# UCF-CRCV/TeD-SPAD

Measured on AMD Instinct MI355X. Metric: clips/sec (16x224^2 I3D features), higher is better.
Workload: dtype f16; 1 GPU; cfg2 dali_extraction path: largei3d extract_features, 225 clip times x 10 crops = 2250 clip-forwards of 3x16x224x224 per GPU per step, random-init weights; global_batch=375, parallelism=clip-sharded x1 + RCCL all-gather of (T,10,F) features

## Files before the change

### ted_spad_amd/csrc/conv_stem_pt.hip

```cpp
#include "conv_common.h"

namespace tedspad {
namespace {

__device__ uint4 g_zero16s;

typedef unsigned u32x4 __attribute__((ext_vector_type(4)));

constexpr int PT_TH = 8, PT_TW = 16;
constexpr int PT_PP = PT_TW + 3;
constexpr int PT_ROWB = 2 * PT_PP * 32;
constexpr int PT_NTAP = 49;
constexpr int PT_W_BYTES = PT_NTAP * 64 * 32;
constexpr int PT_REC = 48;
__host__ __device__ constexpr int pt_rows(int par) { return par == 0 ? PT_TH + 3 : PT_TH + 2; }
__host__ __device__ constexpr int pt_frame(int par) { return pt_rows(par) * PT_ROWB; }
__host__ __device__ constexpr int pt_jobs(int par) { return (2 * pt_frame(par) + 1023) / 1024; }
__host__ __device__ constexpr int pt_off(int par) { return par == 0 ? 0 : pt_jobs(0) * 1024; }
constexpr int PT_W_OFF = pt_off(1) + pt_jobs(1) * 1024;
constexpr int PT_LDS = PT_W_OFF + PT_W_BYTES;
constexpr int PT_NPAIR = 25;
constexpr int PT_W16_BYTES = PT_NPAIR * 64 * 64;
__host__ __device__ constexpr int pt_wbytes(int mf) { return mf == 16 ? PT_W16_BYTES : PT_W_BYTES; }
constexpr int PT_XB_ROW = 9 * 128, PT_XB_BYTES = PT_TH * PT_XB_ROW;
__host__ __device__ constexpr int pt_xb_off(int mf) { return PT_W_OFF + pt_wbytes(mf); }
__host__ __device__ constexpr int pt_lds_pool(int mf) { return pt_xb_off(mf) + PT_XB_BYTES; }
constexpr int PT_LDS_POOL = pt_lds_pool(32);
static_assert(pt_lds_pool(16) <= 160 * 1024 && pt_xb_off(16) % 128 == 0 && pt_xb_off(32) % 128 == 0, "MF = 16 image: exactly 160 KB");
constexpr int PT_POOL_PIECES = 4 * 9 * 8;
static_assert(PT_LDS_POOL <= 160 * 1024, "weights + halo (+ pooled rows) must fit the CU's LDS");
static_assert(PT_W_BYTES % 1024 == 0 && (4 * PT_ROWB) % 256 == 0 && PT_ROWB % 32 == 0, "LDS image alignment");

struct StemPT {
    const unsigned char *x;
    const unsigned char *wimg;
    const float *scale, *shift;
    uint16_t *y;
    long sTp;
    int sH, sP;
    int N, Tp, H, Wq, Ho, Wo, ldy, relu;
// ... 55 lines not shown
        for (int r = 0; r < 2; ++r)
#pragma unroll
            for (int f = 0; f < 2; ++f) xa[r * 2 + f] = *reinterpret_cast<const uint4 *>(dsm + pb[bi] + (pt_off(PAR) + off + f * FR + r * 4 * PT_ROWB));
#pragma unroll
        for (int cb = 0; cb < 2; ++cb) xw[cb] = *reinterpret_cast<const uint4 *>(dsm + wa + (PBASE + i) * 4096 + cb * 1024);
    };
    load(0, fx[0], fw[0]);
    __builtin_amdgcn_sched_group_barrier(0x100, 6, 0);
#pragma unroll
    for (int i = 0; i < NP; ++i) {
        if (i + 1 < NP) load(i + 1, fx[(i + 1) & 1], fw[(i + 1) & 1]);
#pragma unroll
        for (int cb = 0; cb < 2; ++cb)
#pragma unroll
            for (int r = 0; r < 2; ++r)
#pragma unroll
                for (int f = 0; f < 2; ++f) acc[cb][r][f] = T::mfma16(fw[i & 1][cb], fx[i & 1][r * 2 + f], acc[cb][r][f]);
        if (i + 1 < NP) __builtin_amdgcn_sched_group_barrier(0x100, 3, 0);
        __builtin_amdgcn_sched_group_barrier(0x008, 4, 0);
        if (i + 1 < NP) __builtin_amdgcn_sched_group_barrier(0x100, 3, 0);
        __builtin_amdgcn_sched_group_barrier(0x008, 4, 0);
    }
}

template <typename T, int NW, bool POOL, int MF = 32, bool DIRECT = false, int LW = 0>
__global__ __launch_bounds__(64 * (NW + LW)) void conv_stem_pt_kernel(const StemPT p) {
    static_assert(MF == 32 || (MF == 16 && NW == 8 && POOL), "the 16x16x32 form is built for 8 waves with the pool fused");
    static_assert(!DIRECT || (MF == 16 && NW == 8 && POOL), "the fp32-clip loader is built for the production form");
    static_assert(LW == 0 || (MF == 16 && NW == 8 && POOL), "loader waves are built for the production forms");
    constexpr int NA = NW == 8 ? 1 : 2;
    constexpr int XB_OFF = pt_xb_off(MF);
    constexpr int NPT = 64 * (LW ? LW : NW);
    constexpr int PIT = (PT_POOL_PIECES + NPT - 1) / NPT;
    constexpr int NTK = LW ? (4 * pt_rows(0) * 10 + NPT - 1) / NPT : 1;
    constexpr int NLW = LW ? LW : NW;
    constexpr int ROUNDS = (pt_jobs(0) + NLW - 1) / NLW;
    extern __shared__ __attribute__((aligned(16))) unsigned char dsm[];
    const int tid = threadIdx.x, lane = tid & 63;
    const int wave = __builtin_amdgcn_readfirstlane(tid >> 6);
    const int ptid = LW ? tid - 64 * NW : tid;
    const unsigned lds0 = (unsigned)(uintptr_t)(lptr_t)dsm;
    const unsigned char *zero = reinterpret_cast<const unsigned char *>(&g_zero16s);

    const int xcd = blockIdx.x & 7, nx = gridDim.x >> 3;
    const int base = xcd * p.chunk;
    const int lim = min(p.chunk, p.total - base);
    int k = blockIdx.x >> 3;
    if (k >= lim) return;

    if (wave < NW)
        for (int j = wave; j < pt_wbytes(MF) / 1024; j += NW) lds_dma16(p.wimg + j * 1024 + lane * 16, lds0 + PT_W_OFF + j * 1024);

    int off[2][ROUNDS], rc[2][ROUNDS];
    const int dw0 = LW ? wave - NW : wave;
    auto setup_dma = [&]() {
#pragma unroll
    for (int par = 0; par < 2; ++par)
#pragma unroll
        for (int i = 0; i < ROUNDS; ++i) {
            const int s = (i * NLW + dw0) * 64 + lane;
            const int hs = s & 1;
            int q = s >> 1;
            const int pos = q % PT_PP; q /= PT_PP;
            const int b = q & 1; q >>= 1;
            const int row = q % pt_rows(par), f = q / pt_rows(par);
            const int hr = 2 * row + par;
            const int hf = MF == 16 ? hs : hs ^ ((pos >> 3) & 1);
            const bool ok = f < 2;
            off[par][i] = ok ? f * 12 + hf * 16 + hr * p.sH + b * p.sP + (pos - 2) * PT_REC : 0;
            rc[par][i] = ok ? (hr << 8) | pos : (1 << 28);
        }
    };
    if (!DIRECT && !LW) setup_dma();
// ... 8 lines not shown
    auto locate = [&](Patch &q) {
        q.ho0 = q.th * PT_TH; q.wo0 = q.tw * PT_TW;
        q.ih0 = 2 * q.ho0 - 3; q.wqm2 = q.wo0 - 2;
        if (DIRECT) q.pf = p.xf + (long)q.n * p.sN + (long)(4 * q.tp - p.pad_t) * p.sT + (long)q.ih0 * p.sHf + (2 * q.wo0 - 4);
        else q.pb = p.x + ((long)q.n * p.Tp + q.tp) * p.sTp + (long)q.ih0 * p.sH + (long)q.wo0 * PT_REC;
    };
    int dn, dtp, dth, dtw;
    split(nx, dn, dtp, dth, dtw);
    auto advance = [&](const Patch &c) {
        Patch q = c;
        if (POOL && c.th + 1 < p.tiles_h) {
            ++q.th;
            locate(q);
            return q;
        }
        if (POOL) q.th = 0;
        q.tw += dtw; if (q.tw >= p.tiles_w) { q.tw -= p.tiles_w; if (POOL) ++q.tp; else ++q.th; }
        if (!POOL) { q.th += dth; if (q.th >= p.tiles_h) { q.th -= p.tiles_h; ++q.tp; } }
        q.tp += dtp; if (q.tp >= p.Tp) { q.tp -= p.Tp; ++q.n; }
        q.n += dn;
        locate(q);
        return q;
    };
    auto issue = [&](int par, const Patch &q) {
#pragma unroll
        for (int i = 0; i < ROUNDS; ++i) {
            const int j = i * NLW + dw0;
            if (j >= pt_jobs(par)) break;
            const bool ok = (unsigned)(q.ih0 + (rc[par][i] >> 8)) < (unsigned)p.H && (unsigned)(q.wqm2 + (rc[par][i] & 255)) < (unsigned)p.Wq;
            lds_dma16(ok ? q.pb + off[par][i] : zero, lds0 + pt_off(par) + j * 1024);
        }
    };

    int so[2][NTK][LW ? 1 : 8], fsch[2][NTK][2], ldst[2][NTK], dcol[2][NTK], drow[2][NTK];
    f32x4 stage[2][NTK][8];
    auto setup_tasks = [&]() {
#pragma unroll
        for (int par = 0; par < 2; ++par)
#pragma unroll
            for (int t = 0; t < NTK; ++t) {
                const int tk = ptid + t * NPT;
                const int per = pt_rows(par) * 10;
                const int fh = tk / per, rem = tk - fh * per;
                const int row = rem / 10, q4c = rem - row * 10;
                const int f = fh >> 1, hs = fh & 1, hr = 2 * row + par;
                const bool task = fh < 4;
                drow[par][t] = task ? hr : (1 << 20);
                dcol[par][t] = 4 * q4c;
                ldst[par][t] = task ? pt_off(par) + f * pt_frame(par) + row * PT_ROWB + 2 * q4c * 32 + 16 * hs : -1;
                if (LW) { drow[par][t] = (task ? hr : 4095) | (4 * q4c) << 12 | (fh & 3) << 20; dcol[par][t] = 0; so[par][t][0] = hr * p.sHf + 4 * q4c; }
                fsch[par][t][0] = fsch[par][t][1] = 0;
#pragma unroll
                for (int e = 0; e < 8; ++e) {
                    const int v = 6 * f + 8 * hs + e, fs = v / 3, ch = v - 3 * fs;
                    if (!LW) so[par][t][e] = ch * p.sC + fs * p.sT + hr * p.sHf + 4 * q4c;
                    fsch[par][t][e >> 2] |= (fs | (ch << 3)) << (8 * (e & 3));
                }
            }
    };
    if (DIRECT && !LW) setup_tasks();
    auto ldst_of = [&](int par, int t) -> int {
        return ldst[par][t];
    };
    auto issue_d = [&](int par, const Patch &q) {
        const int tt0 = 4 * q.tp - p.pad_t;
#pragma unroll
        for (int t = 0; t < NTK; ++t) {
            int fc0 = fsch[par][t][0], fc1 = fsch[par][t][1], meta = drow[par][t], sb = so[par][t][0];
            if (LW) asm volatile("" : "+v"(meta), "+v"(sb), "+v"(fc0), "+v"(fc1));
            const int t_row = LW ? meta & 4095 : drow[par][t], t_col = LW ? (meta >> 12) & 255 : dcol[par][t];
            const bool rowok = (unsigned)(q.ih0 + t_row) < (unsigned)p.H && (unsigned)(2 * q.wo0 - 4 + t_col) < (unsigned)p.W;
            const bool hs1 = LW ? (t_row != 4095 && ((meta >> 20) & 1)) : (ldst[par][t] >= 0 && ((ldst[par][t] >> 4) & 1));
#pragma unroll
            for (int e = 0; e < 8; ++e) {
                const int code = ((e < 4 ? fc0 : fc1) >> (8 * (e & 3))) & 255;
                const bool ok = rowok && (unsigned)(tt0 + (code & 7)) < (unsigned)p.T && (code >> 3) < p.C && !(e == 7 && hs1);
                const int o = LW ? sb + (code >> 3) * p.sC + (code & 7) * p.sT : so[par][t][e];
                const float *src = ok ? q.pf + o : reinterpret_cast<const float *>(zero);
                unsigned long sa = reinterpret_cast<unsigned long>(src);
                asm volatile("" : "+v"(sa));
                stage[par][t][e] = *reinterpret_cast<const __attribute__((address_space(1))) f32x4 *>(sa);
            }
        }
        asm volatile("" ::: "memory");
    };
    auto cvt2 = [&](float a, float b) -> unsigned {
        if constexpr (T::kDtype == TEDSPAD_F16) {
            unsigned pk;
            const float x = __builtin_amdgcn_fmed3f(a, -65504.f, 65504.f), y = __builtin_amdgcn_fmed3f(b, -65504.f, 65504.f);
            asm("v_cvt_pk_f16_f32 %0, %1, %2" : "=v"(pk) : "v"(x), "v"(y));
            return pk;
        } else {
            return (unsigned)T::from_f32(a) | ((unsigned)T::from_f32(b) << 16);
        }
    };
    auto pack_d = [&](int buf, int t, int j) -> uint4 {
        return make_uint4(cvt2(stage[buf][t][0][j], stage[buf][t][1][j]), cvt2(stage[buf][t][2][j], stage[buf][t][3][j]),
                          cvt2(stage[buf][t][4][j], stage[buf][t][5][j]), cvt2(stage[buf][t][6][j], stage[buf][t][7][j]));
    };
    auto write_d = [&](int par, int t, int j, uint4 v) {
        const bool last = (LW ? (drow[par][t] >> 12) & 255 : dcol[par][t]) == 36;
        const int la = ldst_of(par, t);
        if (la >= 0 && (j < 2 || !last)) *reinterpret_cast<uint4 *>(dsm + la + (j >> 1) * 32 + (j & 1) * (PT_PP * 32)) = v;
    };
    auto commit_d = [&](int par) {
#pragma unroll
        for (int t = 0; t < NTK; ++t)
#pragma unroll
            for (int j = 0; j < 4; ++j) write_d(par, t, j, pack_d(par, t, j));
    };
    Patch cur;
    split(base + k, cur.n, cur.tp, cur.th, cur.tw);
    locate(cur);
    if (DIRECT && !LW) {
        issue_d(0, cur);
        issue_d(1, cur);
        commit_d(0);
        commit_d(1);
    } else if (!DIRECT && !LW) {
        issue(0, cur);
        issue(1, cur);
    }

    auto successor = [&](const Patch &c, int kc, Patch &out, int &kout) -> bool {
        const bool wrap = !POOL || c.th + 1 == p.tiles_h;
        kout = wrap ? kc + nx : kc;
        out = c;
        if (kout >= lim) return false;
        out = advance(c);
        return true;
    };
    const bool dma = !(p.dbg & 1);
    int pxo[PIT], pi[PIT], psl[PIT];
    uint4 carry[PIT];
#pragma unroll
    for (int it = 0; it < PIT; ++it) {
        const int u = ptid + it * NPT;
        psl[it] = (u >> 3) % 9;
        pi[it] = (u >= 0 && u < PT_POOL_PIECES) ? (u >> 3) / 9 : -1;
        pxo[it] = XB_OFF + psl[it] * 128 + (u & 7) * 16;
        carry[it] = make_uint4(0, 0, 0, 0);
    }
    auto pool_rows = [&](const Patch &q) {
        const size_t fr = (size_t)q.n * p.Tp + q.tp;
#pragma unroll
        for (int it = 0; it < PIT; ++it) {
            if (LW) {
                int u = ptid + it * NPT;
                asm volatile("" : "+v"(u));
                psl[it] = (u >> 3) % 9;
                pi[it] = u < PT_POOL_PIECES ? (u >> 3) / 9 : -1;
                pxo[it] = XB_OFF + psl[it] * 128 + (u & 7) * 16;
// ... 20 lines not shown


    if (LW && !DIRECT && wave >= NW) {
        setup_dma();
        Patch c = cur, n1 = cur;
        int kc = k, k1 = 0;
        issue(0, c);
        issue(1, c);
        wait_vmcnt<0>();
        __builtin_amdgcn_s_barrier();
        asm volatile("" ::: "memory");
        while (true) {
            const bool more1 = successor(c, kc, n1, k1);
            wait_vmcnt<0>();
            asm volatile("s_waitcnt lgkmcnt(0)" ::: "memory");
            __builtin_amdgcn_s_barrier();
            asm volatile("" ::: "memory");
            if (more1 && dma) issue(0, n1);
            if (!more1) break;
            wait_vmcnt<0>();
            __builtin_amdgcn_s_barrier();
            asm volatile("" ::: "memory");
            if (dma) issue(1, n1);
            pool_rows(c);
            c = n1; kc = k1;
        }
        asm volatile("; record loaders: last barrier" ::: "memory");
        __builtin_amdgcn_s_barrier();
        asm volatile("" ::: "memory");
        pool_rows(c);
        return;
    }
    if (LW && DIRECT && wave >= NW) {
        setup_tasks();
        Patch c = cur, n1 = cur, n2 = cur;
        int kc = k, k1 = 0, k2 = 0;
        bool more1 = successor(c, kc, n1, k1);
        bool more2 = more1 && successor(n1, k1, n2, k2);
        issue_d(0, c);
        issue_d(1, c);
        wait_vmcnt<0>();
        commit_d(0);
        commit_d(1);
        bool l1 = more1 && dma;
        if (l1) { issue_d(0, n1); issue_d(1, n1); }
        asm volatile("s_waitcnt lgkmcnt(0)" ::: "memory");
        __builtin_amdgcn_s_barrier();
        asm volatile("" ::: "memory");
        while (true) {
            const bool l2 = more2 && dma;
            asm volatile("s_waitcnt lgkmcnt(0)" ::: "memory");
            __builtin_amdgcn_s_barrier();
            asm volatile("" ::: "memory");
            if (l1) {
                wait_vmcnt<8 * NTK>();
                commit_d(0);
                if (l2) issue_d(0, n2);
            }
            if (!more1) break;
            asm volatile("s_waitcnt lgkmcnt(0)" ::: "memory");
            __builtin_amdgcn_s_barrier();
            asm volatile("" ::: "memory");
            if (l1) {
                if (l2) wait_vmcnt<8 * NTK>(); else wait_vmcnt<0>();
                commit_d(1);
                if (l2) issue_d(1, n2);
            }
            pool_rows(c);
            c = n1; kc = k1;
            more1 = more2; n1 = n2; k1 = k2; l1 = l2;
            more2 = more1 && successor(n1, k1, n2, k2);
        }
        asm volatile("; loader waves: last barrier" ::: "memory");
        __builtin_amdgcn_s_barrier();
        asm volatile("" ::: "memory");
        pool_rows(c);
        return;
    }

    const int l15 = lane & 15, rsel = (lane >> 4) & 1, lh = lane >> 5, l31 = lane & 31;
    const int prow = (wave & 3) + 4 * rsel;
    const int a0 = NW == 8 ? wave >> 2 : 0;
    int pa[4], wa[NA];
#pragma unroll
    for (int ta = 0; ta < 4; ++ta) {
        const int pos = l15 + ta;
        pa[ta] = prow * PT_ROWB + pos * 32 + 16 * (lh ^ ((pos >> 3) & 1));
    }
#pragma unroll
    for (int a = 0; a < NA; ++a) wa[a] = PT_W_OFF + ((a0 + a) * 32 + l31) * 32 + 16 * (lh ^ ((((a0 + a) * 32 + l31) >> 4) & 1));

    const int q4 = lane >> 4;
    int pb16[5], wa16 = 0;
    if (MF == 16) {
        const int sel = q4 >> 1, hf = q4 & 1;
#pragma unroll
        for (int j = 0; j < 4; ++j) {
            const int pos = l15 + (j == 3 ? 0 : j + 1);
            const int base = (wave & 3) * PT_ROWB + pos * 32 + 16 * hf;
            pb16[j] = base + sel * (j == 3 ? PT_ROWB : PT_PP * 32);
            if (j == 3) pb16[4] = base;
        }
        const int co0 = a0 * 32 + l15;
        wa16 = PT_W_OFF + co0 * 64 + 16 * (q4 ^ (2 * ((co0 >> 3) & 1)));
    }
    float sc[NA][16], sf[NA][16];
#pragma unroll
    for (int a = 0; a < NA; ++a)
#pragma unroll
        for (int r = 0; r < 16; ++r) {
            const int co = MF == 16 ? a0 * 32 + 16 * ((r >> 2) & 1) + 4 * q4 + (r & 3) : (a0 + a) * 32 + (r & 3) + 8 * (r >> 2) + 4 * lh;
            sc[a][r] = p.scale[co];
            sf[a][r] = p.shift[co];
        }
#pragma unroll
    for (int a = 0; a < NA; ++a)
#pragma unroll
        for (int r = 0; r < 16; ++r) asm volatile("" : "+v"(sc[a][r]), "+v"(sf[a][r]));

    if (DIRECT && !LW && dma) {
        Patch n1; int k1;
        if (successor(cur, k, n1, k1)) { issue_d(0, n1); issue_d(1, n1); }
    }
    wait_vmcnt<0>();
    asm volatile("s_waitcnt lgkmcnt(0)" ::: "memory");
    __builtin_amdgcn_s_barrier();
    asm volatile("" ::: "memory");

    bool pending = false;
    Patch prev = cur;
    while (true) {
        Patch nxt, nn;
        int kn, kn2 = 0;
        const bool more = successor(cur, k, nxt, kn);
        bool more2 = false;
        nn = nxt;
        if (DIRECT && !LW && more) more2 = successor(nxt, kn, nn, kn2);
        if (POOL && !LW && pending) pool_rows(prev);

        f32x16 acc[NA][2];
        f32x4 acc16[2][2][2];
#pragma unroll
        for (int a = 0; a < NA; ++a)
#pragma unroll
            for (int g = 0; g < 2; ++g)
#pragma unroll
                for (int r = 0; r < 16; ++r) acc[a][g][r] = 0.f;
#pragma unroll
        for (int cb = 0; cb < 2; ++cb)
#pragma unroll
            for (int r = 0; r < 2; ++r)
#pragma unroll
                for (int f = 0; f < 2; ++f) acc16[cb][r][f] = f32x4{0.f, 0.f, 0.f, 0.f};

        if (MF == 16) { if (!(p.dbg & 4)) stem_pt_phase16<T, 0>(dsm, pb16, wa16, acc16); }
        else if (!(p.dbg & 4)) stem_pt_phase<T, 0, NA>(dsm, pa, wa, acc);
        if (!DIRECT && !LW) wait_vmcnt<0>();
        else asm volatile("s_waitcnt lgkmcnt(0)" ::: "memory");
        __builtin_amdgcn_s_barrier();
        asm volatile("" ::: "memory");
        if (DIRECT) {
            if (!LW && more && dma) {
                commit_d(0);
                if (more2) issue_d(0, nn);
            }
        } else if (!LW && more && dma) issue(0, nxt);
        if (MF == 16) { if (!(p.dbg & 4)) stem_pt_phase16<T, 1>(dsm, pb16, wa16, acc16); }
        else if (!(p.dbg & 4)) stem_pt_phase<T, 1, NA>(dsm, pa, wa, acc);

        bool stored = false;
        if (POOL && MF == 16) {
#pragma unroll
            for (int r = 0; r < 2; ++r)
#pragma unroll
                for (int cb = 0; cb < 2; ++cb) {
                    float v[4];
#pragma unroll
                    for (int i = 0; i < 4; ++i) {
                        const float s_ = sc[0][4 * cb + i], b_ = sf[0][4 * cb + i];
                        v[i] = __builtin_fmaxf(__builtin_fmaxf(acc16[cb][r][0][i] * s_ + b_, acc16[cb][r][1][i] * s_ + b_), 0.f);
                    }
                    const unsigned d0 = (unsigned)T::from_f32(v[0]) | ((unsigned)T::from_f32(v[1]) << 16);
                    const unsigned d1 = (unsigned)T::from_f32(v[2]) | ((unsigned)T::from_f32(v[3]) << 16);
                    unsigned m[2];
#pragma unroll
                    for (int h = 0; h < 2; ++h) {
                        const unsigned d = h ? d1 : d0;
                        const unsigned s1 = (unsigned)__builtin_amdgcn_update_dpp(0, (int)d, 0x101, 0xf, 0xf, true);
                        const unsigned s2 = (unsigned)__builtin_amdgcn_update_dpp(0, (int)d, 0x102, 0xf, 0xf, true);
                        m[h] = T::pk_max(T::pk_max(d, s1), s2);
                    }
                    unsigned char *xb = dsm + XB_OFF + ((wave & 3) + 4 * r) * PT_XB_ROW + (a0 * 32 + cb * 16 + 4 * q4) * 2;
                    if (!(l15 & 1)) *reinterpret_cast<uint2 *>(xb + (l15 >> 1) * 128) = make_uint2(m[0], m[1]);
                    if (l15 == 0) *reinterpret_cast<uint2 *>(xb + 8 * 128) = make_uint2(d0, d1);
                }
            asm volatile("s_waitcnt lgkmcnt(0)" ::: "memory");
        } else if (POOL) {
#pragma unroll
            for (int a = 0; a < NA; ++a) {
// ... 47 lines not shown
#pragma unroll
            for (int a = 0; a < NA; ++a) {
                unsigned d[4][2];
#pragma unroll
                for (int q = 0; q < 4; ++q)
#pragma unroll
                    for (int h = 0; h < 2; ++h) {
                        float v[2];
#pragma unroll
                        for (int e = 0; e < 2; ++e) {
                            const int r = 4 * q + 2 * h + e;
                            const float v0 = acc[a][0][r] * sc[a][r] + sf[a][r], v1 = acc[a][1][r] * sc[a][r] + sf[a][r];
                            float m = __builtin_fmaxf(v0, v1);
                            if (p.relu) m = __builtin_fmaxf(m, 0.f);
                            v[e] = m;
                        }
                        d[q][h] = (unsigned)T::from_f32(v[0]) | ((unsigned)T::from_f32(v[1]) << 16);
                    }
#pragma unroll
                for (int q = 0; q < 4; q += 2)
#pragma unroll
                    for (int h = 0; h < 2; ++h) {
                        auto sw = __builtin_amdgcn_permlane32_swap(d[q][h], d[q + 1][h], false, false);
                        d[q][h] = sw[0];
                        d[q + 1][h] = sw[1];
                    }
                if (inb) {
                    gstore16(dst + (a0 + a) * 32, u32x4{d[0][0], d[0][1], d[1][0], d[1][1]});
                    gstore16(dst + (a0 + a) * 32 + 16, u32x4{d[2][0], d[2][1], d[3][0], d[3][1]});
                }
            }
        }
        if (!more) break;
        if (DIRECT) asm volatile("s_waitcnt lgkmcnt(0)" ::: "memory");
        else if (LW) asm volatile("s_waitcnt lgkmcnt(0)" ::: "memory");
        else if (stored) wait_vmcnt<2 * NA>(); else wait_vmcnt<0>();
        __builtin_amdgcn_s_barrier();
        asm volatile("" ::: "memory");
        if (DIRECT) {
            if (!LW && dma) {
                commit_d(1);
                if (more2) issue_d(1, nn);
            }
        } else if (!LW && dma) issue(1, nxt);
        prev = cur;
        pending = POOL;
        cur = nxt;
        k = kn;
    }
    if (POOL) {
        __builtin_amdgcn_s_barrier();
        asm volatile("" ::: "memory");
        if (!LW) pool_rows(cur);
    }
}

template <typename T>
__global__ __launch_bounds__(256) void stem_pool_fix_kernel(uint16_t *y, const uint16_t *side, long rows, int wp, int tiles_w, int ldy) {
    const long idx = (long)blockIdx.x * 256 + threadIdx.x;
    const int c8 = (int)(idx & 7);
    const long r = idx >> 3;
    const int tw = 1 + (int)(r % (tiles_w - 1));
    const long row = r / (tiles_w - 1);
    const int pc = 8 * tw - 1;
    if (row >= rows || pc >= wp) return;
    uint4 *d = reinterpret_cast<uint4 *>(y + (row * wp + pc) * ldy + c8 * 8);
    *d = pk_max8<T>(*d, *reinterpret_cast<const uint4 *>(side + (row * tiles_w + tw) * 64 + c8 * 8));
}

template <typename T>
__global__ __launch_bounds__(256) void clip_to_tp_kernel(const float *x, uint16_t *y, int c, int t, int h, int w, long sn, long sc, long st, long sh,
                                                         int pt, int stt, int tp_n, int wtiles) {
    __shared__ __attribute__((aligned(16))) uint4 tile[4 * 2 * 32 * 3];
    const int tid = threadIdx.x, px = tid & 63, grp = tid >> 6;
    int b = blockIdx.x;
    const int wt = b % wtiles; b /= wtiles;
    const int ih = b % h;
// ... 94 lines not shown
        return check_launch("tedspad_clip_to_tp");
    }
    if (dtype == TEDSPAD_F16) hipLaunchKernelGGL(clip_to_tp_kernel<F16>, g, dim3(256), 0, s, x, (uint16_t *)y, c, t, h, w, (long)sn, (long)sc, (long)st, (long)sh, pad_t, stride_t, t_pairs, wtiles);
    else hipLaunchKernelGGL(clip_to_tp_kernel<BF16>, g, dim3(256), 0, s, x, (uint16_t *)y, c, t, h, w, (long)sn, (long)sc, (long)st, (long)sh, pad_t, stride_t, t_pairs, wtiles);
    return check_launch("tedspad_clip_to_tp");
}

extern "C" int32_t tedspad_stem_pt_wimg_bytes(void) { return PT_W_BYTES; }
extern "C" int32_t tedspad_stem_pt_wimg16_bytes(void) { return PT_W16_BYTES; }

static int32_t stem_pt_launch(const char *who, const void *x_tp, const void *w_img, const float *scale, const float *shift, void *y, void *side, int32_t n,
                              int32_t t_pairs, int32_t h, int32_t w, int32_t ho, int32_t wo, int32_t hp, int32_t wp, int32_t ldy, int32_t relu, int32_t nwg,
                              int32_t variant, int32_t dtype, bool pool, hipStream_t s, const StemPT *direct = nullptr) {
    StemPT p;
    p.xf = nullptr; p.sN = 0; p.sC = p.sT = p.sHf = 0; p.C = 3; p.T = 0; p.W = w; p.pad_t = 0;
    if (direct) { p.xf = direct->xf; p.sN = direct->sN; p.sC = direct->sC; p.sT = direct->sT; p.sHf = direct->sHf; p.C = direct->C; p.T = direct->T; p.pad_t = direct->pad_t; }
    p.x = (const unsigned char *)x_tp; p.wimg = (const unsigned char *)w_img; p.scale = scale; p.shift = shift; p.y = (uint16_t *)y;
    p.side = (uint16_t *)side; p.Hp = hp; p.Wp = wp;
    p.Wq = w / 2; p.sP = p.Wq * PT_REC; p.sH = 2 * p.sP; p.sTp = (long)h * p.sH;
    p.N = n; p.Tp = t_pairs; p.H = h; p.Ho = ho; p.Wo = wo; p.ldy = ldy; p.relu = relu;
    p.tiles_h = (ho + PT_TH - 1) / PT_TH; p.tiles_w = (wo + PT_TW - 1) / PT_TW;
    const long total = (long)n * t_pairs * p.tiles_w * (pool ? 1 : p.tiles_h);
    if (total >= (1L << 30) || (long)n * t_pairs * p.tiles_h * p.tiles_w >= (1L << 30)) {
        set_error("%s: too many patches", who);
        return TEDSPAD_EINVAL;
    }
    p.total = (int)total;
    p.chunk = (int)((total + 7) / 8);
    int grid = nwg > 0 ? nwg : 256;
    grid = (grid + 7) / 8 * 8;
    if ((long)grid > total + 7) grid = (int)((total + 7) / 8 * 8);
    static thread_local int attr_set[8] = {0, 0, 0, 0, 0, 0, 0, 0};
    const int w8 = (variant >> 1) & 1;
    p.dbg = (variant >> 8) & 15;
    if (direct) {
        static const bool lw = getenv("TEDSPAD_STEM_LOADERS") == nullptr || atoi(getenv("TEDSPAD_STEM_LOADERS")) != 0;
        static thread_local int attrd[4] = {0, 0, 0, 0};
        const int ti = (dtype == TEDSPAD_F16 ? 0 : 1) + (lw ? 2 : 0);
        const void *fnd = ti == 0 ? (const void *)conv_stem_pt_kernel<F16, 8, true, 16, true> : ti == 1 ? (const void *)conv_stem_pt_kernel<BF16, 8, true, 16, true>
                        : ti == 2 ? (const void *)conv_stem_pt_kernel<F16, 8, true, 16, true, 8> : (const void *)conv_stem_pt_kernel<BF16, 8, true, 16, true, 8>;
        if (!attrd[ti]) {
            if (hipFuncSetAttribute(fnd, hipFuncAttributeMaxDynamicSharedMemorySize, 160 * 1024) != hipSuccess) {
                set_error("%s: cannot raise the dynamic LDS limit", who);
                return TEDSPAD_ELAUNCH;
            }
            attrd[ti] = 1;
        }
        if (ti == 0) hipLaunchKernelGGL((conv_stem_pt_kernel<F16, 8, true, 16, true>), dim3(grid), dim3(512), pt_lds_pool(16), s, p);
        else if (ti == 1) hipLaunchKernelGGL((conv_stem_pt_kernel<BF16, 8, true, 16, true>), dim3(grid), dim3(512), pt_lds_pool(16), s, p);
        else if (ti == 2) hipLaunchKernelGGL((conv_stem_pt_kernel<F16, 8, true, 16, true, 8>), dim3(grid), dim3(1024), pt_lds_pool(16), s, p);
        else hipLaunchKernelGGL((conv_stem_pt_kernel<BF16, 8, true, 16, true, 8>), dim3(grid), dim3(1024), pt_lds_pool(16), s, p);
    } else if (pool && (variant & 4)) {
        static const bool lw = getenv("TEDSPAD_STEM_LOADERS") == nullptr || atoi(getenv("TEDSPAD_STEM_LOADERS")) != 0;
        static thread_local int attr16[4] = {0, 0, 0, 0};
        const int ti = (dtype == TEDSPAD_F16 ? 0 : 1) + (lw ? 2 : 0);
        const void *fn16 = ti == 0 ? (const void *)conv_stem_pt_kernel<F16, 8, true, 16> : ti == 1 ? (const void *)conv_stem_pt_kernel<BF16, 8, true, 16>
                         : ti == 2 ? (const void *)conv_stem_pt_kernel<F16, 8, true, 16, false, 4> : (const void *)conv_stem_pt_kernel<BF16, 8, true, 16, false, 4>;
        if (!attr16[ti]) {
            if (hipFuncSetAttribute(fn16, hipFuncAttributeMaxDynamicSharedMemorySize, 160 * 1024) != hipSuccess) {
                set_error("%s: cannot raise the dynamic LDS limit", who);
                return TEDSPAD_ELAUNCH;
            }
            attr16[ti] = 1;
        }
        if (ti == 0) hipLaunchKernelGGL((conv_stem_pt_kernel<F16, 8, true, 16>), dim3(grid), dim3(512), pt_lds_pool(16), s, p);
        else if (ti == 1) hipLaunchKernelGGL((conv_stem_pt_kernel<BF16, 8, true, 16>), dim3(grid), dim3(512), pt_lds_pool(16), s, p);
        else if (ti == 2) hipLaunchKernelGGL((conv_stem_pt_kernel<F16, 8, true, 16, false, 4>), dim3(grid), dim3(768), pt_lds_pool(16), s, p);
        else hipLaunchKernelGGL((conv_stem_pt_kernel<BF16, 8, true, 16, false, 4>), dim3(grid), dim3(768), pt_lds_pool(16), s, p);
    } else {
    const int di = ((dtype == TEDSPAD_F16 ? 0 : 1) * 2 + w8) * 2 + (pool ? 1 : 0);
    const void *fns[8] = {(const void *)conv_stem_pt_kernel<F16, 4, false>, (const void *)conv_stem_pt_kernel<F16, 4, true>,
                          (const void *)conv_stem_pt_kernel<F16, 8, false>, (const void *)conv_stem_pt_kernel<F16, 8, true>,
                          (const void *)conv_stem_pt_kernel<BF16, 4, false>, (const void *)conv_stem_pt_kernel<BF16, 4, true>,
                          (const void *)conv_stem_pt_kernel<BF16, 8, false>, (const void *)conv_stem_pt_kernel<BF16, 8, true>};
    if (!attr_set[di]) {
        if (hipFuncSetAttribute(fns[di], hipFuncAttributeMaxDynamicSharedMemorySize, 160 * 1024) != hipSuccess) {
            set_error("%s: cannot raise the dynamic LDS limit", who);
            return TEDSPAD_ELAUNCH;
        }
        attr_set[di] = 1;
    }
    const dim3 g(grid), b(w8 ? 512 : 256);
    const int lds = pool ? PT_LDS_POOL : PT_LDS;
// ... 26 lines not shown
    TS_REQUIRE(ldy >= 64 && ldy % 8 == 0 && ((uintptr_t)x_tp | (uintptr_t)w_img | (uintptr_t)y) % 16 == 0, "tedspad_stem_pt_fwd: 64 output channels, 16-byte aligned pointers");
    TS_REQUIRE(dtype == TEDSPAD_F16 || dtype == TEDSPAD_BF16, "tedspad_stem_pt_fwd: bad dtype");
    TS_REQUIRE((long)h * w * PT_REC < (1L << 31), "tedspad_stem_pt_fwd: frame too large for 32-bit halo offsets");
    return stem_pt_launch("tedspad_stem_pt_fwd", x_tp, w_img, scale, shift, y, nullptr, n, t_pairs, h, w, ho, wo, 0, 0, ldy, relu, nwg, variant, dtype, false,
                          (hipStream_t)stream);
}

extern "C" int64_t tedspad_stem_pt_side_bytes(int32_t n, int32_t t_pairs, int32_t h, int32_t w) {
    const int ho = (h + 1) / 2, wo = w / 2;
    if (n <= 0 || t_pairs <= 0 || ho < 3 || wo < 3) return 0;
    return (int64_t)n * t_pairs * ((ho - 3) / 2 + 1) * ((wo + PT_TW - 1) / PT_TW) * 64 * 2;
}

extern "C" int32_t tedspad_stem_pt_pool_fwd(const void *x_tp, const void *w_img, const float *scale, const float *shift, void *y, void *side, int32_t n,
                                            int32_t t_pairs, int32_t h, int32_t w, int32_t hp, int32_t wp, int32_t ldy, int32_t nwg, int32_t variant,
                                            int32_t dtype, void *stream) {
    TS_REQUIRE(x_tp && w_img && scale && shift && y && side && n > 0 && t_pairs > 0 && h > 0 && w > 0 && w % 2 == 0, "tedspad_stem_pt_pool_fwd: bad arguments");
    const int ho = (h + 1) / 2, wo = w / 2;
    TS_REQUIRE(ho >= 3 && wo >= 3 && hp == (ho - 3) / 2 + 1 && wp == (wo - 3) / 2 + 1, "tedspad_stem_pt_pool_fwd: 3x3 stride-2 unpadded pool of the ceil(h/2) x w/2 stem output");
    TS_REQUIRE(ldy >= 64 && ldy % 8 == 0 && ((uintptr_t)x_tp | (uintptr_t)w_img | (uintptr_t)y | (uintptr_t)side) % 16 == 0, "tedspad_stem_pt_pool_fwd: 64 output channels, 16-byte aligned pointers");
    TS_REQUIRE(dtype == TEDSPAD_F16 || dtype == TEDSPAD_BF16, "tedspad_stem_pt_pool_fwd: bad dtype");
    TS_REQUIRE((long)h * w * PT_REC < (1L << 31), "tedspad_stem_pt_pool_fwd: frame too large for 32-bit halo offsets");
    return stem_pt_launch("tedspad_stem_pt_pool_fwd", x_tp, w_img, scale, shift, y, side, n, t_pairs, h, w, ho, wo, hp, wp, ldy, 1, nwg, variant, dtype, true,
                          (hipStream_t)stream);
}

extern "C" int32_t tedspad_stem_pt_pool_clip_fwd(const float *x, int32_t n, int32_t c, int32_t t, int32_t h, int32_t w, int64_t sn, int64_t sc, int64_t st, int64_t sh,
                                                 int64_t sw, int32_t pad_t, int32_t stride_t, int32_t t_pairs, const void *w_img16, const float *scale,
                                                 const float *shift, void *y, void *side, int32_t hp, int32_t wp, int32_t ldy, int32_t nwg, int32_t variant,
                                                 int32_t dtype, void *stream) {
    TS_REQUIRE(x && w_img16 && scale && shift && y && side && n > 0 && c > 0 && c <= 3 && t > 0 && h > 0 && w > 0 && t_pairs > 0 && pad_t >= 0,
               "tedspad_stem_pt_pool_clip_fwd: bad arguments");
    TS_REQUIRE(stride_t == 2, "tedspad_stem_pt_pool_clip_fwd: temporal stride 2");
    TS_REQUIRE(h < 4000 && w < 8000, "tedspad_stem_pt_pool_clip_fwd: frames up to 4000 x 8000 (the loader's packed task word)");
    TS_REQUIRE(sw == 1 && w % 4 == 0 && ((uintptr_t)x | (uintptr_t)(sn * 4) | (uintptr_t)(sc * 4) | (uintptr_t)(st * 4) | (uintptr_t)(sh * 4)) % 16 == 0,
               "tedspad_stem_pt_pool_clip_fwd: rows must be contiguous and 16-byte aligned (w %% 4 == 0, strides multiples of 4 elements)");
    TS_REQUIRE(sc >= 0 && st >= 0 && sh >= 0 && sn >= 0 && (c - 1) * sc + (long)(t + 8) * st + (long)(h + 32) * sh + w + 64 < (1L << 31),
               "tedspad_stem_pt_pool_clip_fwd: a sample must fit 32-bit element offsets");
    const int ho = (h + 1) / 2, wo = w / 2;
    TS_REQUIRE(ho >= 3 && wo >= 3 && hp == (ho - 3) / 2 + 1 && wp == (wo - 3) / 2 + 1, "tedspad_stem_pt_pool_clip_fwd: 3x3 stride-2 unpadded pool of the ceil(h/2) x w/2 stem output");
    TS_REQUIRE(ldy >= 64 && ldy % 8 == 0 && ((uintptr_t)w_img16 | (uintptr_t)y | (uintptr_t)side) % 16 == 0, "tedspad_stem_pt_pool_clip_fwd: 64 output channels, 16-byte aligned pointers");
    TS_REQUIRE(dtype == TEDSPAD_F16 || dtype == TEDSPAD_BF16, "tedspad_stem_pt_pool_clip_fwd: bad dtype");
    StemPT d;
    d.xf = x; d.sN = (long)sn; d.sC = (int)sc; d.sT = (int)st; d.sHf = (int)sh; d.C = c; d.T = t; d.pad_t = pad_t;
    return stem_pt_launch("tedspad_stem_pt_pool_clip_fwd", nullptr, w_img16, scale, shift, y, side, n, t_pairs, h, w, ho, wo, hp, wp, ldy, 1, nwg, variant | 6, dtype, true,
                          (hipStream_t)stream, &d);
}
```

### ted_spad_amd/engine.py

```python
from __future__ import annotations

import ctypes as C
import os
import weakref
from dataclasses import dataclass
from typing import Optional, Tuple

import torch

from . import _lib
from ._lib import ConvDesc, PoolDesc, check

DTYPES = {"f16": (torch.float16, _lib.F16), "bf16": (torch.bfloat16, _lib.BF16)}
DEFAULT_DTYPE = "f16"

BNECK_FRAME = os.environ.get("TEDSPAD_BNECK_FRAME", "1") != "0"
BNECK_TAIL = os.environ.get("TEDSPAD_BNECK_TAIL", "1") != "0"
BNECK_TAIL128 = os.environ.get("TEDSPAD_BNECK_TAIL128", "1") != "0"
BNECK_TAIL_POOL = os.environ.get("TEDSPAD_BNECK_TAIL_POOL", "1") != "0"
TPAIR_MIN_COUT = int(os.environ.get("TEDSPAD_TPAIR_MIN_COUT", "128"))
TPAIR = os.environ.get("TEDSPAD_TPAIR", "1") != "0"
STEM_POOL = os.environ.get("TEDSPAD_STEM_POOL", "1") != "0"
UPP_TAIL = os.environ.get("TEDSPAD_UPP_TAIL", "1") != "0"
GATHER_CAT = os.environ.get("TEDSPAD_GATHER_CAT", "1") != "0"
# ... 873 lines not shown

    def conv(self, xtp: torch.Tensor, relu=True, variant=None) -> Act:
        n, tp, h, _, wq, _ = xtp.shape
        w = 2 * wq
        ho, wo = (h + 1) // 2, wq
        out = Act.empty(n, tp, ho, wo, 64, self.torch_dtype, xtp.device)
        check(_lib.lib().tedspad_stem_pt_fwd(xtp.data_ptr(), self.wimg.data_ptr(), self.scale.data_ptr(), self.shift.data_ptr(), out.ptr, n, tp, h, w,
                                             ho, wo, out.ld, int(relu), self.nwg, (self.VARIANT if variant is None else variant) & ~4,
                                             self.dtype_code, _stream_ptr()), "tedspad_stem_pt_fwd")
        return out

    def conv_pool(self, xtp: torch.Tensor, variant=None) -> Act:
        n, tp, h, _, wq, _ = xtp.shape
        w = 2 * wq
        ho, wo = (h + 1) // 2, wq
        assert ho >= 3 and wo >= 3, "StemPT.conv_pool: the stem output must hold one 3x3 window"
        hp, wp = (ho - 3) // 2 + 1, (wo - 3) // 2 + 1
        out = Act.empty(n, tp, hp, wp, 64, self.torch_dtype, xtp.device)
        side = torch.empty(_lib.lib().tedspad_stem_pt_side_bytes(n, tp, h, w), dtype=torch.uint8, device=xtp.device)
        v = self.VARIANT if variant is None else variant
        if v & 4:
            v |= 2
        check(_lib.lib().tedspad_stem_pt_pool_fwd(xtp.data_ptr(), (self.wimg16 if v & 4 else self.wimg).data_ptr(), self.scale.data_ptr(), self.shift.data_ptr(),
                                                  out.ptr, side.data_ptr(), n, tp, h, w, hp, wp, out.ld, self.nwg, v, self.dtype_code, _stream_ptr()),
              "tedspad_stem_pt_pool_fwd")
        return out

    def direct_applies(self, x: torch.Tensor) -> bool:
        if not (self.applies(x) and x.dtype == torch.float32 and x.shape[4] % 4 == 0 and x.data_ptr() % 16 == 0):
            return False
        n, c, t, h, w = x.shape
        sn, sc, st, sh, _ = x.stride()
        return (all(s_ % 4 == 0 and s_ >= 0 for s_ in (sn, sc, st, sh)) and (c - 1) * sc + (t + 8) * st + (h + 32) * sh + w + 64 < (1 << 31) and
                (h + 1) // 2 >= 3 and w // 2 >= 3)

    def conv_pool_clip(self, x: torch.Tensor, variant=0) -> Act:
        require_cuda(x, "StemPT")
        n, c, t, h, w = x.shape
        tp = self.frame_pairs(t)
        ho, wo = (h + 1) // 2, w // 2
        hp, wp = (ho - 3) // 2 + 1, (wo - 3) // 2 + 1
        out = Act.empty(n, tp, hp, wp, 64, self.torch_dtype, x.device)
        side = torch.empty(_lib.lib().tedspad_stem_pt_side_bytes(n, tp, h, w), dtype=torch.uint8, device=x.device)
        sn, sc, st, sh, sw = x.stride()
        check(_lib.lib().tedspad_stem_pt_pool_clip_fwd(x.data_ptr(), n, c, t, h, w, sn, sc, st, sh, sw, self.pad_t, self.stride_t, tp, self.wimg16.data_ptr(),
                                                       self.scale.data_ptr(), self.shift.data_ptr(), out.ptr, side.data_ptr(), hp, wp, out.ld, self.nwg,
                                                       variant, self.dtype_code, _stream_ptr()), "tedspad_stem_pt_pool_clip_fwd")
        return out

    def __call__(self, x: torch.Tensor, relu=True) -> Act:
        return self.conv(self.layout(x), relu)


def act_to_nchw(x: Act, c: Optional[int] = None) -> torch.Tensor:
    n, t, h, w = x.dims
    c = x.c if c is None else c
    y = torch.empty((n, c, t, h, w), dtype=torch.float32, device=x.buf.device)
    code = _lib.F16 if x.buf.dtype == torch.float16 else _lib.BF16
    check(_lib.lib().tedspad_channels_last_to_nchw(x.ptr, y.data_ptr(), n, c, t, h, w, x.ld, code, _stream_ptr()),
          "tedspad_channels_last_to_nchw")
    return y


def upsample2x_into(x: Act, out: Act, pad_top=0, pad_left=0):
    n, t, h, w = x.dims
    no, to, ho, wo = out.dims
    assert t == 1 and to == 1 and no == n and out.c == x.c
# ... 5 lines not shown
```

Baseline: 24500 clips/s.

## Specialize fp32-clip stem loader waves by task kind and drop non-loader direct path

Restructures the fp32-clip stem loader so each pair of loader waves handles one fixed slice of the frame/channel planes, a compile-time kind chosen through a template constant. This cuts per-element packed task words and repeated address decoding. When a patch lies fully inside the frame it uses a fast unpredicated load path, and one kind reuses packed values to fill two overlapping LDS slots. It also removes the direct variant without loader waves and the TEDSPAD_STEM_LOADERS switch, and adds a row-stride bound check on both host and Python sides. Risks are register pressure from the per-kind code and lost coverage for configurations that used the removed variant.

```diff
diff --git a/ted_spad_amd/csrc/conv_stem_pt.hip b/ted_spad_amd/csrc/conv_stem_pt.hip
--- a/ted_spad_amd/csrc/conv_stem_pt.hip
+++ b/ted_spad_amd/csrc/conv_stem_pt.hip
@@ -6,6 +6,7 @@
 __device__ uint4 g_zero16s;
 
 typedef unsigned u32x4 __attribute__((ext_vector_type(4)));
+template <int K> struct IntC { static constexpr int value = K; };
 
 constexpr int PT_TH = 8, PT_TW = 16;
 constexpr int PT_PP = PT_TW + 3;
@@ -127,13 +128,12 @@
     constexpr int XB_OFF = pt_xb_off(MF);
     constexpr int NPT = 64 * (LW ? LW : NW);
     constexpr int PIT = (PT_POOL_PIECES + NPT - 1) / NPT;
-    constexpr int NTK = LW ? (4 * pt_rows(0) * 10 + NPT - 1) / NPT : 1;
     constexpr int NLW = LW ? LW : NW;
     constexpr int ROUNDS = (pt_jobs(0) + NLW - 1) / NLW;
     extern __shared__ __attribute__((aligned(16))) unsigned char dsm[];
     const int tid = threadIdx.x, lane = tid & 63;
     const int wave = __builtin_amdgcn_readfirstlane(tid >> 6);
-    const int ptid = LW ? tid - 64 * NW : tid;
+    int ptid = LW ? tid - 64 * NW : tid;
     const unsigned lds0 = (unsigned)(uintptr_t)(lptr_t)dsm;
     const unsigned char *zero = reinterpret_cast<const unsigned char *>(&g_zero16s);
 
@@ -208,58 +208,6 @@
         }
     };
 
-    int so[2][NTK][LW ? 1 : 8], fsch[2][NTK][2], ldst[2][NTK], dcol[2][NTK], drow[2][NTK];
-    f32x4 stage[2][NTK][8];
-    auto setup_tasks = [&]() {
-#pragma unroll
-        for (int par = 0; par < 2; ++par)
-#pragma unroll
-            for (int t = 0; t < NTK; ++t) {
-                const int tk = ptid + t * NPT;
-                const int per = pt_rows(par) * 10;
-                const int fh = tk / per, rem = tk - fh * per;
-                const int row = rem / 10, q4c = rem - row * 10;
-                const int f = fh >> 1, hs = fh & 1, hr = 2 * row + par;
-                const bool task = fh < 4;
-                drow[par][t] = task ? hr : (1 << 20);
-                dcol[par][t] = 4 * q4c;
-                ldst[par][t] = task ? pt_off(par) + f * pt_frame(par) + row * PT_ROWB + 2 * q4c * 32 + 16 * hs : -1;
-                if (LW) { drow[par][t] = (task ? hr : 4095) | (4 * q4c) << 12 | (fh & 3) << 20; dcol[par][t] = 0; so[par][t][0] = hr * p.sHf + 4 * q4c; }
-                fsch[par][t][0] = fsch[par][t][1] = 0;
-#pragma unroll
-                for (int e = 0; e < 8; ++e) {
-                    const int v = 6 * f + 8 * hs + e, fs = v / 3, ch = v - 3 * fs;
-                    if (!LW) so[par][t][e] = ch * p.sC + fs * p.sT + hr * p.sHf + 4 * q4c;
-                    fsch[par][t][e >> 2] |= (fs | (ch << 3)) << (8 * (e & 3));
-                }
-            }
-    };
-    if (DIRECT && !LW) setup_tasks();
-    auto ldst_of = [&](int par, int t) -> int {
-        return ldst[par][t];
-    };
-    auto issue_d = [&](int par, const Patch &q) {
-        const int tt0 = 4 * q.tp - p.pad_t;
-#pragma unroll
-        for (int t = 0; t < NTK; ++t) {
-            int fc0 = fsch[par][t][0], fc1 = fsch[par][t][1], meta = drow[par][t], sb = so[par][t][0];
-            if (LW) asm volatile("" : "+v"(meta), "+v"(sb), "+v"(fc0), "+v"(fc1));
-            const int t_row = LW ? meta & 4095 : drow[par][t], t_col = LW ? (meta >> 12) & 255 : dcol[par][t];
-            const bool rowok = (unsigned)(q.ih0 + t_row) < (unsigned)p.H && (unsigned)(2 * q.wo0 - 4 + t_col) < (unsigned)p.W;
-            const bool hs1 = LW ? (t_row != 4095 && ((meta >> 20) & 1)) : (ldst[par][t] >= 0 && ((ldst[par][t] >> 4) & 1));
-#pragma unroll
-            for (int e = 0; e < 8; ++e) {
-                const int code = ((e < 4 ? fc0 : fc1) >> (8 * (e & 3))) & 255;
-                const bool ok = rowok && (unsigned)(tt0 + (code & 7)) < (unsigned)p.T && (code >> 3) < p.C && !(e == 7 && hs1);
-                const int o = LW ? sb + (code >> 3) * p.sC + (code & 7) * p.sT : so[par][t][e];
-                const float *src = ok ? q.pf + o : reinterpret_cast<const float *>(zero);
-                unsigned long sa = reinterpret_cast<unsigned long>(src);
-                asm volatile("" : "+v"(sa));
-                stage[par][t][e] = *reinterpret_cast<const __attribute__((address_space(1))) f32x4 *>(sa);
-            }
-        }
-        asm volatile("" ::: "memory");
-    };
     auto cvt2 = [&](float a, float b) -> unsigned {
         if constexpr (T::kDtype == TEDSPAD_F16) {
             unsigned pk;
@@ -270,30 +218,10 @@
             return (unsigned)T::from_f32(a) | ((unsigned)T::from_f32(b) << 16);
         }
     };
-    auto pack_d = [&](int buf, int t, int j) -> uint4 {
-        return make_uint4(cvt2(stage[buf][t][0][j], stage[buf][t][1][j]), cvt2(stage[buf][t][2][j], stage[buf][t][3][j]),
-                          cvt2(stage[buf][t][4][j], stage[buf][t][5][j]), cvt2(stage[buf][t][6][j], stage[buf][t][7][j]));
-    };
-    auto write_d = [&](int par, int t, int j, uint4 v) {
-        const bool last = (LW ? (drow[par][t] >> 12) & 255 : dcol[par][t]) == 36;
-        const int la = ldst_of(par, t);
-        if (la >= 0 && (j < 2 || !last)) *reinterpret_cast<uint4 *>(dsm + la + (j >> 1) * 32 + (j & 1) * (PT_PP * 32)) = v;
-    };
-    auto commit_d = [&](int par) {
-#pragma unroll
-        for (int t = 0; t < NTK; ++t)
-#pragma unroll
-            for (int j = 0; j < 4; ++j) write_d(par, t, j, pack_d(par, t, j));
-    };
     Patch cur;
     split(base + k, cur.n, cur.tp, cur.th, cur.tw);
     locate(cur);
-    if (DIRECT && !LW) {
-        issue_d(0, cur);
-        issue_d(1, cur);
-        commit_d(0);
-        commit_d(1);
-    } else if (!DIRECT && !LW) {
+    if (!LW) {
         issue(0, cur);
         issue(1, cur);
     }
@@ -380,49 +308,119 @@
         return;
     }
     if (LW && DIRECT && wave >= NW) {
-        setup_tasks();
-        Patch c = cur, n1 = cur, n2 = cur;
-        int kc = k, k1 = 0, k2 = 0;
-        bool more1 = successor(c, kc, n1, k1);
-        bool more2 = more1 && successor(n1, k1, n2, k2);
-        issue_d(0, c);
-        issue_d(1, c);
-        wait_vmcnt<0>();
-        commit_d(0);
-        commit_d(1);
-        bool l1 = more1 && dma;
-        if (l1) { issue_d(0, n1); issue_d(1, n1); }
-        asm volatile("s_waitcnt lgkmcnt(0)" ::: "memory");
-        __builtin_amdgcn_s_barrier();
-        asm volatile("" ::: "memory");
-        while (true) {
-            const bool l2 = more2 && dma;
+        static_assert(!DIRECT || LW == 8, "the fp32-clip loader: four wave pairs, one task kind each");
+        ptid = 64 * (wave - NW) + (int)__builtin_amdgcn_mbcnt_hi(~0u, __builtin_amdgcn_mbcnt_lo(~0u, 0u));
+        const int kind = (wave - NW) >> 1;
+        auto run = [&](auto KIND) {
+            constexpr int KD = decltype(KIND)::value;
+            constexpr int V0 = KD == 0 ? 0 : KD == 1 ? 6 : 14;
+            constexpr int NL = KD == 0 ? 8 : KD == 1 ? 9 : KD == 2 ? 7 : 0;
+            const int rem = ptid & 127, row = rem / 10, q4c = rem - row * 10;
+            unsigned voff[2];
+            int ldst[2];
+#pragma unroll
+            for (int par = 0; par < 2; ++par) {
+                const bool task = NL > 0 && row < pt_rows(par);
+                voff[par] = task ? ((unsigned)((2 * row + par) * p.sHf) + 4u * q4c) * 4u : 0u;
+                ldst[par] = task ? pt_off(par) + row * PT_ROWB + q4c * 64 : -1;
+            }
+            f32x4 stage[2][NL ? NL : 1];
+            auto issue_d = [&](int par, const Patch &q) {
+                const int tt0 = 4 * q.tp - p.pad_t;
+                unsigned valid = 0;
+#pragma unroll
+                for (int e = 0; e < NL; ++e) {
+                    const int v = V0 + e, fs = v / 3, ch = v - 3 * fs;
+                    valid |= (unsigned)((unsigned)(tt0 + fs) < (unsigned)p.T && ch < p.C) << e;
+                }
+                const bool allv = valid == (1u << NL) - 1;
+                auto plane = [&](int e) -> int { const int v = V0 + e, fs = v / 3, ch = v - 3 * fs; return ch * p.sC + fs * p.sT; };
+                const bool inside = q.ih0 >= 0 && q.ih0 + 20 < p.H && q.wo0 >= 2 && 2 * q.wo0 + 32 < p.W;
+                if (inside && allv && !(p.dbg & 16)) {
+                    if (ldst[par] >= 0) {
+#pragma unroll
+                        for (int e = 0; e < NL; ++e) {
+                            const unsigned char *sb = reinterpret_cast<const unsigned char *>(q.pf + plane(e));
+                            stage[par][e] = *reinterpret_cast<const __attribute__((address_space(1))) f32x4 *>(reinterpret_cast<unsigned long>(sb) + voff[par]);
+                        }
+                    }
+                } else {
+                    const bool okrc = ldst[par] >= 0 && (unsigned)(q.ih0 + 2 * row + par) < (unsigned)p.H && (unsigned)(2 * q.wo0 - 4 + 4 * q4c) < (unsigned)p.W && !(p.dbg & 16);
+#pragma unroll
+                    for (int e = 0; e < NL; ++e) {
+                        const unsigned char *src = okrc && ((valid >> e) & 1) ? reinterpret_cast<const unsigned char *>(q.pf + plane(e)) + voff[par] : zero;
+                        unsigned long sa = reinterpret_cast<unsigned long>(src);
+                        asm volatile("" : "+v"(sa));
+                        stage[par][e] = *reinterpret_cast<const __attribute__((address_space(1))) f32x4 *>(sa);
+                    }
+                }
+                asm volatile("" ::: "memory");
+            };
+            auto commit_d = [&](int par) {
+                if (NL == 0 || ldst[par] < 0 || (p.dbg & 8)) return;
+                const f32x4 (&sg)[NL ? NL : 1] = stage[par];
+#pragma unroll
+                for (int j = 0; j < 4; ++j) {
+                    if (j >= 2 && q4c == 9) break;
+                    unsigned char *d = dsm + ldst[par] + (j >> 1) * 32 + (j & 1) * (PT_PP * 32);
+                    if constexpr (KD == 0) {
+                        *reinterpret_cast<uint4 *>(d) = make_uint4(cvt2(sg[0][j], sg[1][j]), cvt2(sg[2][j], sg[3][j]), cvt2(sg[4][j], sg[5][j]), cvt2(sg[6][j], sg[7][j]));
+                    } else if constexpr (KD == 1) {
+                        const unsigned p3 = cvt2(sg[0][j], sg[1][j]), p4 = cvt2(sg[2][j], sg[3][j]), p5 = cvt2(sg[4][j], sg[5][j]), p6 = cvt2(sg[6][j], sg[7][j]);
+                        *reinterpret_cast<uint4 *>(d + pt_frame(par)) = make_uint4(p3, p4, p5, p6);
+                        *reinterpret_cast<uint4 *>(d + 16) = make_uint4(p4, p5, p6, cvt2(sg[8][j], 0.f));
+                    } else if constexpr (KD == 2) {
+                        *reinterpret_cast<uint4 *>(d + pt_frame(par) + 16) = make_uint4(cvt2(sg[0][j], sg[1][j]), cvt2(sg[2][j], sg[3][j]), cvt2(sg[4][j], sg[5][j]), cvt2(sg[6][j], 0.f));
+                    }
+                }
+            };
+            Patch c = cur, n1 = cur, n2 = cur;
+            int kc = k, k1 = 0, k2 = 0;
+            bool more1 = successor(c, kc, n1, k1);
+            bool more2 = more1 && successor(n1, k1, n2, k2);
+            issue_d(0, c);
+            issue_d(1, c);
+            wait_vmcnt<0>();
+            commit_d(0);
+            commit_d(1);
+            bool l1 = more1 && dma;
+            if (l1) { issue_d(0, n1); issue_d(1, n1); }
             asm volatile("s_waitcnt lgkmcnt(0)" ::: "memory");
             __builtin_amdgcn_s_barrier();
             asm volatile("" ::: "memory");
-            if (l1) {
-                wait_vmcnt<8 * NTK>();
-                commit_d(0);
-                if (l2) issue_d(0, n2);
-            }
-            if (!more1) break;
-            asm volatile("s_waitcnt lgkmcnt(0)" ::: "memory");
+            while (true) {
+                const bool l2 = more2 && dma;
+                asm volatile("s_waitcnt lgkmcnt(0)" ::: "memory");
+                __builtin_amdgcn_s_barrier();
+                asm volatile("" ::: "memory");
+                if (l1) {
+                    wait_vmcnt<NL>();
+                    commit_d(0);
+                    if (l2) issue_d(0, n2);
+                }
+                if (!more1) break;
+                asm volatile("s_waitcnt lgkmcnt(0)" ::: "memory");
+                __builtin_amdgcn_s_barrier();
+                asm volatile("" ::: "memory");
+                if (l1) {
+                    if (l2) wait_vmcnt<NL>(); else wait_vmcnt<0>();
+                    commit_d(1);
+                    if (l2) issue_d(1, n2);
+                }
+                pool_rows(c);
+                c = n1; kc = k1;
+                more1 = more2; n1 = n2; k1 = k2; l1 = l2;
+                more2 = more1 && successor(n1, k1, n2, k2);
+            }
+            asm volatile("; loader waves: last barrier" ::: "memory");
             __builtin_amdgcn_s_barrier();
             asm volatile("" ::: "memory");
-            if (l1) {
-                if (l2) wait_vmcnt<8 * NTK>(); else wait_vmcnt<0>();
-                commit_d(1);
-                if (l2) issue_d(1, n2);
-            }
             pool_rows(c);
-            c = n1; kc = k1;
-            more1 = more2; n1 = n2; k1 = k2; l1 = l2;
-            more2 = more1 && successor(n1, k1, n2, k2);
-        }
-        asm volatile("; loader waves: last barrier" ::: "memory");
-        __builtin_amdgcn_s_barrier();
-        asm volatile("" ::: "memory");
-        pool_rows(c);
+        };
+        if (kind == 0) run(IntC<0>{});
+        else if (kind == 1) run(IntC<1>{});
+        else if (kind == 2) run(IntC<2>{});
+        else run(IntC<3>{});
         return;
     }
 
@@ -466,10 +464,6 @@
 #pragma unroll
         for (int r = 0; r < 16; ++r) asm volatile("" : "+v"(sc[a][r]), "+v"(sf[a][r]));
 
-    if (DIRECT && !LW && dma) {
-        Patch n1; int k1;
-        if (successor(cur, k, n1, k1)) { issue_d(0, n1); issue_d(1, n1); }
-    }
     wait_vmcnt<0>();
     asm volatile("s_waitcnt lgkmcnt(0)" ::: "memory");
     __builtin_amdgcn_s_barrier();
@@ -478,12 +472,9 @@
     bool pending = false;
     Patch prev = cur;
     while (true) {
-        Patch nxt, nn;
-        int kn, kn2 = 0;
+        Patch nxt;
+        int kn;
         const bool more = successor(cur, k, nxt, kn);
-        bool more2 = false;
-        nn = nxt;
-        if (DIRECT && !LW && more) more2 = successor(nxt, kn, nn, kn2);
         if (POOL && !LW && pending) pool_rows(prev);
 
         f32x16 acc[NA][2];
@@ -503,16 +494,11 @@
 
         if (MF == 16) { if (!(p.dbg & 4)) stem_pt_phase16<T, 0>(dsm, pb16, wa16, acc16); }
         else if (!(p.dbg & 4)) stem_pt_phase<T, 0, NA>(dsm, pa, wa, acc);
-        if (!DIRECT && !LW) wait_vmcnt<0>();
+        if (!LW) wait_vmcnt<0>();
         else asm volatile("s_waitcnt lgkmcnt(0)" ::: "memory");
         __builtin_amdgcn_s_barrier();
         asm volatile("" ::: "memory");
-        if (DIRECT) {
-            if (!LW && more && dma) {
-                commit_d(0);
-                if (more2) issue_d(0, nn);
-            }
-        } else if (!LW && more && dma) issue(0, nxt);
+        if (!LW && more && dma) issue(0, nxt);
         if (MF == 16) { if (!(p.dbg & 4)) stem_pt_phase16<T, 1>(dsm, pb16, wa16, acc16); }
         else if (!(p.dbg & 4)) stem_pt_phase<T, 1, NA>(dsm, pa, wa, acc);
 
@@ -626,17 +612,11 @@
             }
         }
         if (!more) break;
-        if (DIRECT) asm volatile("s_waitcnt lgkmcnt(0)" ::: "memory");
-        else if (LW) asm volatile("s_waitcnt lgkmcnt(0)" ::: "memory");
+        if (LW) asm volatile("s_waitcnt lgkmcnt(0)" ::: "memory");
         else if (stored) wait_vmcnt<2 * NA>(); else wait_vmcnt<0>();
         __builtin_amdgcn_s_barrier();
         asm volatile("" ::: "memory");
-        if (DIRECT) {
-            if (!LW && dma) {
-                commit_d(1);
-                if (more2) issue_d(1, nn);
-            }
-        } else if (!LW && dma) issue(1, nxt);
+        if (!LW && dma) issue(1, nxt);
         prev = cur;
         pending = POOL;
         cur = nxt;
@@ -797,13 +777,11 @@
     if ((long)grid > total + 7) grid = (int)((total + 7) / 8 * 8);
     static thread_local int attr_set[8] = {0, 0, 0, 0, 0, 0, 0, 0};
     const int w8 = (variant >> 1) & 1;
-    p.dbg = (variant >> 8) & 15;
+    p.dbg = (variant >> 8) & 31;
     if (direct) {
-        static const bool lw = getenv("TEDSPAD_STEM_LOADERS") == nullptr || atoi(getenv("TEDSPAD_STEM_LOADERS")) != 0;
-        static thread_local int attrd[4] = {0, 0, 0, 0};
-        const int ti = (dtype == TEDSPAD_F16 ? 0 : 1) + (lw ? 2 : 0);
-        const void *fnd = ti == 0 ? (const void *)conv_stem_pt_kernel<F16, 8, true, 16, true> : ti == 1 ? (const void *)conv_stem_pt_kernel<BF16, 8, true, 16, true>
-                        : ti == 2 ? (const void *)conv_stem_pt_kernel<F16, 8, true, 16, true, 8> : (const void *)conv_stem_pt_kernel<BF16, 8, true, 16, true, 8>;
+        static thread_local int attrd[2] = {0, 0};
+        const int ti = dtype == TEDSPAD_F16 ? 0 : 1;
+        const void *fnd = ti == 0 ? (const void *)conv_stem_pt_kernel<F16, 8, true, 16, true, 8> : (const void *)conv_stem_pt_kernel<BF16, 8, true, 16, true, 8>;
         if (!attrd[ti]) {
             if (hipFuncSetAttribute(fnd, hipFuncAttributeMaxDynamicSharedMemorySize, 160 * 1024) != hipSuccess) {
                 set_error("%s: cannot raise the dynamic LDS limit", who);
@@ -811,9 +789,7 @@
             }
             attrd[ti] = 1;
         }
-        if (ti == 0) hipLaunchKernelGGL((conv_stem_pt_kernel<F16, 8, true, 16, true>), dim3(grid), dim3(512), pt_lds_pool(16), s, p);
-        else if (ti == 1) hipLaunchKernelGGL((conv_stem_pt_kernel<BF16, 8, true, 16, true>), dim3(grid), dim3(512), pt_lds_pool(16), s, p);
-        else if (ti == 2) hipLaunchKernelGGL((conv_stem_pt_kernel<F16, 8, true, 16, true, 8>), dim3(grid), dim3(1024), pt_lds_pool(16), s, p);
+        if (ti == 0) hipLaunchKernelGGL((conv_stem_pt_kernel<F16, 8, true, 16, true, 8>), dim3(grid), dim3(1024), pt_lds_pool(16), s, p);
         else hipLaunchKernelGGL((conv_stem_pt_kernel<BF16, 8, true, 16, true, 8>), dim3(grid), dim3(1024), pt_lds_pool(16), s, p);
     } else if (pool && (variant & 4)) {
         static const bool lw = getenv("TEDSPAD_STEM_LOADERS") == nullptr || atoi(getenv("TEDSPAD_STEM_LOADERS")) != 0;
@@ -906,7 +882,7 @@
     TS_REQUIRE(x && w_img16 && scale && shift && y && side && n > 0 && c > 0 && c <= 3 && t > 0 && h > 0 && w > 0 && t_pairs > 0 && pad_t >= 0,
                "tedspad_stem_pt_pool_clip_fwd: bad arguments");
     TS_REQUIRE(stride_t == 2, "tedspad_stem_pt_pool_clip_fwd: temporal stride 2");
-    TS_REQUIRE(h < 4000 && w < 8000, "tedspad_stem_pt_pool_clip_fwd: frames up to 4000 x 8000 (the loader's packed task word)");
+    TS_REQUIRE(h < 4000 && w < 8000 && sh < (1L << 25), "tedspad_stem_pt_pool_clip_fwd: frames up to 4000 x 8000, rows up to 2^25 elements apart (the loader's 32-bit byte offset inside a halo)");
     TS_REQUIRE(sw == 1 && w % 4 == 0 && ((uintptr_t)x | (uintptr_t)(sn * 4) | (uintptr_t)(sc * 4) | (uintptr_t)(st * 4) | (uintptr_t)(sh * 4)) % 16 == 0,
                "tedspad_stem_pt_pool_clip_fwd: rows must be contiguous and 16-byte aligned (w %% 4 == 0, strides multiples of 4 elements)");
     TS_REQUIRE(sc >= 0 && st >= 0 && sh >= 0 && sn >= 0 && (c - 1) * sc + (long)(t + 8) * st + (long)(h + 32) * sh + w + 64 < (1L << 31),
diff --git a/ted_spad_amd/engine.py b/ted_spad_amd/engine.py
--- a/ted_spad_amd/engine.py
+++ b/ted_spad_amd/engine.py
@@ -929,7 +929,7 @@
         n, c, t, h, w = x.shape
         sn, sc, st, sh, _ = x.stride()
         return (all(s_ % 4 == 0 and s_ >= 0 for s_ in (sn, sc, st, sh)) and (c - 1) * sc + (t + 8) * st + (h + 32) * sh + w + 64 < (1 << 31) and
-                (h + 1) // 2 >= 3 and w // 2 >= 3)
+                (h + 1) // 2 >= 3 and w // 2 >= 3 and h < 4000 and w < 8000 and sh < (1 << 25))
 
     def conv_pool_clip(self, x: torch.Tensor, variant=0) -> Act:
         require_cuda(x, "StemPT")
```

Result: no change. 24290 clips/s (-0.9%).
